# Robin-Lenoir/replication-social-bank-runs

Hardware: AMD Instinct MI355X
Metric: equilibria solved/sec on β×u grid (FP64) (higher is better)
Workload: dtype f64; 1 GPU; fig5_beta_u_sweep_2048x2048_per_gpu (BASELINE config 3); n_beta_per_gpu=2048, n_u=2048, early_exit=False, parallelism=beta-column shards x1, beta_axis_columns=2048, pipelined=True

## Files before the change

### include/sbr.h

```cpp
#ifndef SBR_H
#define SBR_H

#include <stdint.h>

#include "sbr_status.h"

#ifdef __cplusplus
extern "C" {
#endif

#define SBR_OK 0
#define SBR_EARG (-1)
#define SBR_EDEVICE (-2)
#define SBR_ENOMEM (-3)

typedef struct sbr_ctx sbr_ctx;

typedef struct {
    double ode_reltol;
    double ode_abstol;
    int64_t ode_maxiters;
    int32_t bisect_max_iters;
    int32_t early_exit_nan_run;
    int32_t knot_capacity;
    int32_t hetero_max_iters;
    int32_t flags;
    int32_t pad;
    double xi_guess;
} sbr_opts;

#define SBR_FLAG_EXHAUSTIVE 0x1
#define SBR_FLAG_READY_SWEEP 0x2
#define SBR_FLAG_RCCL_GATHER 0x4
#define SBR_FLAG_XI_GUESS 0x8
#define SBR_FLAG_DIAG_STOP_AFTER_BUFFER 0x100
#define SBR_FLAG_DIAG_STOP_AFTER_BISECT 0x200
#define SBR_FLAG_DIAG_COUNT_AW_BLOCKS 0x400
#define SBR_FLAG_DIAG_SOCIAL_PROF 0x800
#define SBR_FLAG_DIAG_NO_AW_WINDOW 0x1000
#define SBR_FLAG_HETERO_WIDE 0x2000

#define SBR_HETERO_MAX_K 16

typedef struct {
    double* xi;
    double* tau_in_unc;
    double* tau_out_unc;
    double* aw_max;
    double* tol;
    uint32_t* status;
    int32_t* iters;
} sbr_result_soa;

void sbr_default_opts(sbr_opts* o);

int sbr_init(int device, sbr_ctx** ctx);
int sbr_free(sbr_ctx* ctx);
const char* sbr_last_error(const sbr_ctx* ctx);

int sbr_init_multi(int n_gpus, const int* devices, sbr_ctx** ctx);
int sbr_multi_size(const sbr_ctx* ctx);
sbr_ctx* sbr_multi_child(sbr_ctx* ctx, int rank);

// ... 138 lines not shown
```

### replication-social-bank-runs_amd/csrc/sbr_baseline.hip

```cpp
#include "sbr_device.h"
#include "sbr_hazard_dev.h"
#include "sbr_kernels.h"
#include "sbr_ode.h"
#include "sbr_point_dev.h"
#include "sbr_scan.h"
#include "sbr_solve_dev.h"

namespace sbr {

constexpr int kLearnBlock = 128;
constexpr int kLearnBlockLat = 64;

__device__ __forceinline__ void publish_column(const LearnArgs& a, int b)
{
    const int k = atomicAdd(a.ready_tail, 1);
    __hip_atomic_store(a.ready_q + k, b + 1, __ATOMIC_RELEASE, __HIP_MEMORY_SCOPE_AGENT);
}
#define st_knot(p, v) (*(p) = (v))
constexpr int kStageSlots = 24;
constexpr size_t kStageLdsPerWave = (size_t)4 * kStageSlots * 64 * sizeof(double);
template <int LB, bool STAGE = false>
__global__ __launch_bounds__(LB) void learn_logistic_kernel(const double* __restrict__ beta,
                                                            const double* __restrict__ eta,
                                                            const double* __restrict__ t_end, LearnArgs a,
// ... 256 lines not shown
    double tin, tout;
    if (!any) {
        tin = T1; tout = T1;
    } else if (all) {
        tin = tau(0); tout = tau(ntau - 1);
    } else {
        tin = T1; tout = T1;
        if (cin >= 0) {
            const double t0 = tau(cin), t1 = tau(cin + 1), h0 = H[cin], h1 = H[cin + 1];
            tin = t0 + ((u - h0) * (t1 - t0)) / (h1 - h0);
        }
        if (cout >= 0) {
            const double t0 = tau(cout), t1 = tau(cout + 1), h0 = H[cout], h1 = H[cout + 1];
            tout = t0 + ((u - h0) * (t1 - t0)) / (h1 - h0);
        }
        if (tin == T1) tin = tau(fa);
        if (tout == T1) tout = tau(la);
    }
    r.tin = tin;
    r.tout = tout;
    if (diag & 1) return;
    solve_from_buffers(T, G, H, S, n, ntau, nle, ETA, T1, trunc, u, kappa, max_iters, lbits, r, aw_path, diag,
                       tin, tout);
}

template <class P>
__device__ __forceinline__ void solve_from_buffers(P T, P G, P H, const Summ& S, const int n, const int ntau,
                                                   const int nle, const double ETA, const double T1, const bool trunc,
                                                   const double u, const double kappa, const int max_iters,
                                                   const uint32_t lbits, PointResult& r, double* __restrict__ aw_path,
                                                   const int diag, const double tin, const double tout)
{
    const double tlo = T[0], thi = T[n - 1];
    auto tau = [&](int i) -> double { return i < nle ? T[i] : ETA; };
    if (tin == tout) {
        r.status = SBR_NO_RUN_HR_BELOW_U | SBR_CONVERGED | lbits;
        r.tol = 0.0;
        return;
    }

    uint32_t flag = 0;
    const double tolerance = 10.0 * sbr_jl_eps(kappa);
    double xnew = (tin + tout) / 2.0, xmin = tin, xmax = tout;
    const bool okmin = in_range(xmin, tlo, thi, trunc, flag);
    const bool okmax = in_range(xmax, tlo, thi, trunc, flag);
    if (!okmin || !okmax) {
// ... 410 lines not shown
        r.tin = NAN; r.tout = NAN;
        return;
    }
    sv.finish();
    const int ns = sv.nh;
    double tin, tout;
    if (!sv.any) {
        tin = T1; tout = T1;
    } else if (sv.all) {
        tin = tau[0]; tout = tau[ns - 1];
    } else {
        tin = sv.cin >= 0 ? sv.tin_x : T1;
        tout = sv.cout >= 0 ? sv.tout_x : T1;
        if (tin == T1) tin = tau[sv.fa];
        if (tout == T1) tout = tau[sv.la];
    }
    r.tin = tin;
    r.tout = tout;
    if (diag & 1) { r.status = bits; return; }
    solve_from_buffers(T, G, H, S, n, ntau, nle, ETA, T1, trunc, u, kappa, max_iters, bits, r, aw_path, diag, tin,
                       tout);
}

template <int BLOCK, bool INTEREST, int MODE = 0>
__device__ __forceinline__ void eq_column(const int b, const int j0, const int j1, const LearnBufs& L,
                                          const double* __restrict__ eta, const double* __restrict__ t_end,
                                          const double* __restrict__ u, const EqArgs& a, const InterestArgs& ia,
                                          const ResultSoA& out, double* smem)
{
    const int n = L.n_knots[b], ntau = L.n_tau[b], nle = L.n_le[b];
    const uint32_t lst = L.status[b];
    const size_t row = (size_t)b * (size_t)L.cap;
    const double* __restrict__ gT = L.t + row;
    const double* __restrict__ gG = L.G + row;
    const double* __restrict__ gH = L.hr + row;
    constexpr int NS = INTEREST ? 3 : 2;
    const bool fits = n <= a.lds_cap && (!INTEREST || ntau <= a.lds_cap);
    if ((MODE == 1 && !fits) || (MODE == 2 && fits)) return;
    double* sT = smem;
    double* sG = smem + a.lds_cap;
    double* sH = INTEREST ? smem + 2 * a.lds_cap : nullptr;
    const double* __restrict__ cH = INTEREST ? sH : gH;
    const int nsum = (a.lds_cap >> 6) + 1, nsum8 = (a.lds_cap >> 3) + 1;
    double* hmax = smem + NS * a.lds_cap;
    double* hmin = hmax + nsum;
    double* pmc = hmin + nsum;
    double* smc = pmc + nsum8;
    double* hpm = smc + nsum8;
    double* hpn = hpm + nsum;
    double* hsm = hpn + nsum;
    double* hsn = hsm + nsum;
    const int nbh_s = (ntau + 63) >> 6;
    __shared__ int eq_next;
    __shared__ int s_nonmono;
    __shared__ int s_noscan;
    __shared__ int s_near1;
    __shared__ int s_ndec;
    __shared__ unsigned long long s_maxdec;
    __shared__ double s_thalf;
    __shared__ int s_wb;
    __shared__ unsigned long long s_dmax;
    if (threadIdx.x == 0) { eq_next = 0; s_nonmono = 0; s_noscan = 0; s_near1 = 0; s_ndec = 0; s_maxdec = 0; s_thalf = NAN; s_wb = 0x7fffffff; s_dmax = 0; }
    if (fits) {
        for (int i = threadIdx.x; i < n; i += BLOCK) { sT[i] = gT[i]; sG[i] = gG[i]; }
        if (INTEREST)
            for (int i = threadIdx.x; i < ntau; i += BLOCK) sH[i] = gH[i];
    }
    __syncthreads();
    Summ S{nullptr, nullptr, nullptr, nullptr, false, (double)NAN, false, 0.0, false, 2, nullptr, nullptr, nullptr,
           nullptr, 0};
    if (fits && !a.exhaustive) {
        const int nbh = (ntau + 63) >> 6, nbg = (n + 7) >> 3;
        const int nq = nbh << 3;
        for (int bk = threadIdx.x; bk < nq + nbg; bk += BLOCK) {
            if (bk < nq) {
                double mx = -INFINITY, mn = INFINITY;
                const int i0 = bk << 3;
                double h[8];
#pragma unroll
                for (int k = 0; k < 8; k++) h[k] = i0 + k < ntau ? cH[i0 + k] : -INFINITY;
#pragma unroll
                for (int k = 0; k < 8; k++) {
                    if (i0 + k >= ntau) continue;
                    if (h[k] > mx) mx = h[k];
                    mn = (h[k] != h[k]) ? -INFINITY : (h[k] < mn ? h[k] : mn);
                }
#pragma unroll
                for (int off = 1; off < 8; off <<= 1) {
                    const double omx = __shfl_xor(mx, off, 8), omn = __shfl_xor(mn, off, 8);
                    mx = omx > mx ? omx : mx;
                    mn = omn < mn ? omn : mn;
                }
                if ((bk & 7) == 0) {
                    hmax[bk >> 3] = mx;
                    hmin[bk >> 3] = mn;
                }
            } else {
                const int g = bk - nq;
                double mx = -INFINITY, mn = INFINITY;
                const int e = (g << 3) + 8 < n ? (g << 3) + 8 : n;
                double prev = g > 0 ? sG[(g << 3) - 1] : -INFINITY;
                bool mono = true, nan = false;
                int ndec = 0;
                double maxdec = 0.0;
                for (int i = g << 3; i < e; i++) {
                    const double v = sG[i];
                    if (v != v) { mx = NAN; mn = NAN; mono = false; nan = true; break; }
                    if (v > mx) mx = v;
                    if (v < mn) mn = v;
                    const bool dec = v < prev;
                    mono &= !dec;
                    ndec += dec ? 1 : 0;
                    maxdec = dec && prev - v > maxdec ? prev - v : maxdec;
                    prev = v;
                }
                if (!mono) s_nonmono = 1;
                if (nan) s_noscan = 1;
                if (ndec) {
                    atomicAdd(&s_ndec, ndec);
                    atomicMax(&s_maxdec, (unsigned long long)sbr_dbits(maxdec));
                }
                const double sep = 1e-15 * sT[n - 1];
                bool far = true, far1 = true;
                for (int i = g << 3; i < e; i++) {
                    far &= i + 2 >= n || sT[i + 2] - sT[i] > sep;
                    far1 &= i + 1 >= n || sT[i + 1] - sT[i] > sep;
                }
                if (!far) s_noscan = 1;
                if (!far1) s_near1 = 1;
                pmc[g] = mx;
                smc[g] = mn;
            }
        }
        {
            auto rises = [](double lo, double hi) {
                const double m = fabs(lo) > fabs(hi) ? fabs(lo) : fabs(hi);
                return m >= 0x1p-900 && m <= 1e300 && hi - lo > 0x1p-50 * m;
            };
            const int ln = threadIdx.x & 63;
            for (int q = threadIdx.x >> 6; q * 62 < n - 1; q += BLOCK >> 6) {
                const int k = q * 62 + ln - 2;
                const bool valid = k >= 0 && k <= n - 2;
                const double d = valid ? (sG[k + 1] - sG[k]) / (sT[k + 1] - sT[k]) : 0.0;
                const double d1 = __shfl_up(d, 1, 64);
                const bool inc = rises(d1, d), dec = rises(d, d1);
                const bool incp = __shfl_up((int)inc, 1, 64) != 0;
                const bool mine = valid && ln >= 2;
                const bool fail = mine && k >= 1 && ((!inc && !dec) || (k >= 2 && inc && !incp));
                double ad = mine ? fabs(d) : 0.0;
                ad = ad <= 1e300 ? ad : (double)INFINITY;
#pragma unroll
                for (int off = 1; off < 64; off <<= 1) {
                    const double o = __shfl_xor(ad, off, 64);
                    ad = o > ad ? o : ad;
                }
                const unsigned long long fm = __ballot(fail);
                if (ln == 0) {
                    if (fm) atomicMin(&s_wb, q * 62 + (int)__builtin_ctzll(fm) - 2);
                    atomicMax(&s_dmax, (unsigned long long)sbr_dbits(ad));
                }
            }
        }
        __syncthreads();
        if (threadIdx.x == 0) {
            int lo = 0, hi = n - 1;
            if (n >= 2 && sG[0] <= 0.5 && sG[n - 1] > 0.5) {
                while (hi - lo > 1) {
                    const int mid = (lo + hi) >> 1;
                    if (sG[mid] <= 0.5) lo = mid;
                    else hi = mid;
                }
                s_thalf = sT[lo] + (0.5 - sG[lo]) * (sT[hi] - sT[lo]) / (sG[hi] - sG[lo]);
            }
            if (s_nonmono && s_noscan)
            for (int g = 1; g < nbg; g++) {
                const double a0 = pmc[g - 1], b0 = pmc[g];
                pmc[g] = (a0 != a0 || b0 != b0) ? NAN : (a0 > b0 ? a0 : b0);
            }
        } else if (threadIdx.x == (BLOCK > 64 ? 64 : 1) && s_nonmono && s_noscan) {
            for (int g = nbg - 2; g >= 0; g--) {
                const double a0 = smc[g + 1], b0 = smc[g];
                smc[g] = (a0 != a0 || b0 != b0) ? NAN : (a0 < b0 ? a0 : b0);
            }
        }
        if (BLOCK >= 256 && (threadIdx.x >> 6) >= 2 && (threadIdx.x >> 6) <= 3) {
            const bool fwd = (threadIdx.x >> 6) == 2;
            const int ln = threadIdx.x & 63;
            double ca = -INFINITY, cb = INFINITY;
            for (int c0 = 0; c0 < nbh; c0 += 64) {
                const int g = fwd ? c0 + ln : nbh - 1 - c0 - ln;
                const bool in = fwd ? g < nbh : g >= 0;
                double a = in ? hmax[g] : -INFINITY, b = in ? hmin[g] : INFINITY;
                for (int off = 1; off < 64; off <<= 1) {
                    const double oa = __shfl_up(a, off, 64), ob = __shfl_up(b, off, 64);
                    if (ln >= off) { a = oa > a ? oa : a; b = ob < b ? ob : b; }
                }
                a = ca > a ? ca : a;
                b = cb < b ? cb : b;
                if (in) {
                    if (fwd) { hpm[g] = a; hpn[g] = b; }
                    else { hsm[g] = a; hsn[g] = b; }
                }
                ca = __shfl(a, 63, 64);
                cb = __shfl(b, 63, 64);
            }
        }
        if (BLOCK < 256 && threadIdx.x == 2) {
            double a0 = -INFINITY, b0 = INFINITY;
            for (int g = 0; g < nbh; g++) {
                a0 = hmax[g] > a0 ? hmax[g] : a0;
                b0 = hmin[g] < b0 ? hmin[g] : b0;
                hpm[g] = a0;
                hpn[g] = b0;
            }
        }
        if (BLOCK < 256 && threadIdx.x == 3) {
            double a0 = -INFINITY, b0 = INFINITY;
            for (int g = nbh - 1; g >= 0; g--) {
                a0 = hmax[g] > a0 ? hmax[g] : a0;
                b0 = hmin[g] < b0 ? hmin[g] : b0;
                hsm[g] = a0;
                hsn[g] = b0;
            }
        }
        __syncthreads();
        auto uni = [](double x) {
            const unsigned long long v = sbr_dbits(x);
            const unsigned lo = __builtin_amdgcn_readfirstlane((unsigned)v);
            const unsigned hi = __builtin_amdgcn_readfirstlane((unsigned)(v >> 32));
            return sbr_bitsd(((unsigned long long)hi << 32) | lo);
        };
        const double dd = uni((double)s_ndec * sbr_bitsd(s_maxdec));
        S = Summ{hmax, hmin, pmc, smc, s_nonmono == 0, uni(s_thalf),
                 n >= 2 && !s_noscan && dd <= 1e-12 && sG[0] >= 0.0 && sG[n - 1] <= 2.0, dd,
                 s_nonmono == 0 || s_noscan != 0, s_near1 == 0 ? 1 : 2,
                 hpm, hpn, hsm, hsn, nbh_s};
        const double dmax = sbr_bitsd(s_dmax);
        if (n >= 2 && dmax <= 1e300 && !(a.diag & 16)) {
            const int wb = s_wb < n - 1 ? s_wb : n - 1;
            const double e0 = fabs(sT[0]), e1 = fabs(sT[n - 1]);
            const double span = (sT[wb] + 2.0 * (e0 > e1 ? e0 : e1)) * (1.0 + 0x1p-40);
            const double du = 0x1p-52 * span;
            const double wm = 0x1p-46 + dmax * (0x1p-50 * span);
            if (wm <= 1e-9) {
                S.wlo = uni((sT[0] > 0.0 ? sT[0] : 0.0) + du);
                S.whi = uni(sT[wb] - du);
                S.wm = uni(wm);
            }
        }
    }
    const int lane = threadIdx.x & 63;
    const double ETA = eta[b], T1 = t_end[b];
    const uint32_t lbits = lst & (SBR_ODE_MAXITERS | SBR_STIFF_SWITCH | SBR_ODE_FAILED | SBR_KNOT_OVERFLOW);
    const bool bad_col = (lst & (SBR_ARG_INVALID | SBR_OOB)) || n < 2;
    const bool trunc = !a.full_grid && n >= 2 && gT[n - 1] < T1 && !(lst & kLearnCutBits);
    for (;;) {
        int base = 0;
        if (lane == 0) base = atomicAdd(&eq_next, 64);
        base = __builtin_amdgcn_readfirstlane(base);
        if (j0 + base >= j1) break;
        const int j = j0 + base + lane;
        if (j >= j1) continue;
        const double uj = u[j];
        PointResult r;
        int64_t vsteps = 0;
        if (bad_col || !(uj >= 0.0)) {
            r.xi = NAN; r.aw = NAN; r.tol = INFINITY; r.iters = 0;
            r.tin = NAN; r.tout = NAN;
            r.status = ((lst & SBR_ARG_INVALID) || !(uj >= 0.0)) ? SBR_ARG_INVALID : (SBR_OOB | lbits);
        } else if (INTEREST && ia.r > 0.0) {
            if (MODE != 2 && fits)
                solve_interest_point(sT, sG, sH, S, n, ntau, nle, ETA, T1, trunc, uj, a.kappa, a.max_iters, lbits, ia,
                                     r, vsteps, a.aw_path, a.diag);
            else if (MODE != 1)
                solve_interest_point(gT, gG, gH, S, n, ntau, nle, ETA, T1, trunc, uj, a.kappa, a.max_iters, lbits, ia,
                                     r, vsteps, a.aw_path, a.diag);
        } else if (MODE != 2 && fits) {
            solve_point((const double*)sT, (const double*)sG, cH, S, n, ntau, nle, ETA, T1, trunc, uj, a.kappa,
// ... 229 lines not shown

hipError_t launch_learn_logistic(const double* beta, const double* eta, const double* t_end, const LearnArgs& a,
                                 const LearnBufs& L, hipStream_t s)
{
    hipError_t e = launch_learn_kernel(beta, eta, t_end, a, L, s, (a.fuse_hazard && !a.ready_q) ? 0 : 1);
    if (e != hipSuccess) return e;
    if (a.ready_q) return hipSuccess;
    if (a.fuse_hazard) return launch_hazard_norm(a, L, a.n_beta, s);
    hipLaunchKernelGGL(hazard_kernel, dim3(a.n_beta), dim3(HZ_BLOCK), 0, s, beta,
                       eta, a, L);
    return hipGetLastError();
}

hipError_t launch_hazard(const double* beta, const double* eta, const LearnArgs& a, const LearnBufs& L, int n_beta,
                         hipStream_t s)
{
    hipLaunchKernelGGL(hazard_kernel, dim3(n_beta), dim3(HZ_BLOCK), 0, s, beta, eta, a, L);
    return hipGetLastError();
}

hipError_t launch_equilibrium(const LearnBufs& L, const double* eta, const double* t_end, const double* u,
                              const EqArgs& a, const ResultSoA& out, int n_beta, hipStream_t s, int only_mode)
{
    const size_t lds = ((size_t)2 * a.lds_cap + 6 * ((a.lds_cap >> 6) + 1) + 2 * ((a.lds_cap >> 3) + 1)) * sizeof(double);
    const int tiles = (a.n_u + EQ_TILE - 1) / EQ_TILE;
    const int w = a.n_u < EQ_TILE ? a.n_u : EQ_TILE;
    dim3 grid(tiles, n_beta);
    const InterestArgs none{0.0, 1.0, 0.0, 0.0, 0, nullptr, nullptr, nullptr};
    auto go = [&](auto k1, auto k2, int bs) {
        if (only_mode != 2) hipLaunchKernelGGL(k1, grid, dim3(bs), lds, s, L, eta, t_end, u, a, none, out);
        if (only_mode != 1) hipLaunchKernelGGL(k2, grid, dim3(bs), 0, s, L, eta, t_end, u, a, none, out);
    };
    if (w > 256)
        go(equilibrium_kernel<kEqWide, false, 1>, equilibrium_kernel<kEqWide, false, 2>, kEqWide);
    else if (w > 64)
        go(equilibrium_kernel<256, false, 1>, equilibrium_kernel<256, false, 2>, 256);
    else
        go(equilibrium_kernel<64, false, 1>, equilibrium_kernel<64, false, 2>, 64);
    return hipGetLastError();
}

hipError_t launch_eq_ready(const LearnBufs& L, const double* beta, const double* eta, const double* t_end,
                           const double* u, const LearnArgs& la, const EqArgs& a, const ReadyArgs& ra,
                           const ResultSoA& out, int n_blocks, hipStream_t s)
{
    size_t lds = ((size_t)2 * a.lds_cap + 6 * ((a.lds_cap >> 6) + 1) + 2 * ((a.lds_cap >> 3) + 1)) * sizeof(double);
    const size_t hz = (size_t)(3 * HZ_LDS + 3) * sizeof(double);
    if (lds < hz) lds = hz;
    (void)n_blocks;
    hipLaunchKernelGGL(eq_ready_kernel, dim3(ra.n_items), dim3(kEqWide), lds, s, L, beta, eta, t_end, u, la, a, ra,
                       out);
    return hipGetLastError();
}

__global__ __launch_bounds__(256) void ready_fail_kernel(const int32_t* __restrict__ gave_up, ResultSoA out,
                                                          int64_t n_pts)
{
    if (__hip_atomic_load(gave_up, __ATOMIC_RELAXED, __HIP_MEMORY_SCOPE_AGENT) == 0) return;
    for (int64_t i = (int64_t)blockIdx.x * 256 + threadIdx.x; i < n_pts; i += (int64_t)gridDim.x * 256) {
        out.xi[i] = NAN;
        out.tau_in_unc[i] = NAN;
        out.tau_out_unc[i] = NAN;
        out.aw_max[i] = NAN;
        out.tol[i] = INFINITY;
        out.status[i] = SBR_ENGINE_SCHED;
        if (out.iters) out.iters[i] = 0;
    }
}

hipError_t launch_ready_fail(const int32_t* gave_up, const ResultSoA& out, int64_t n_pts, hipStream_t s)
{
    hipLaunchKernelGGL(ready_fail_kernel, dim3(256), dim3(256), 0, s, gave_up, out, n_pts);
// ... 37 lines not shown
```

### replication-social-bank-runs_amd/csrc/sbr_capi.hip

```cpp
#include <math.h>
#include <stdio.h>
#include <stdlib.h>
#include <string.h>

#include <algorithm>
#include <array>
#include <chrono>
#include <string>
#include <thread>
#include <vector>

#include "../../include/sbr.h"
#include "../../include/sbr_detmath.h"
#include "sbr_hostcopy.h"
#include "sbr_kernels.h"
#include "sbr_multi.h"
#include "sbr_social_plan.h"

constexpr unsigned kTimingEventFlags = hipEventDisableSystemFence;
constexpr unsigned kSyncEventFlags = hipEventDisableTiming | hipEventReleaseToDevice;



struct sbr_ctx {
// ... 377 lines not shown

hipEvent_t tstart(sbr_ctx* c, hipStream_t s)
{
    if (!c->timing) return nullptr;
    hipEvent_t e = next_event(c);
    if (e) (void)hipEventRecord(e, s);
    return e;
}

void tend(sbr_ctx* c, hipStream_t s, int kind, hipEvent_t a, int count = 1)
{
    if (!c->timing || !a) return;
    hipEvent_t e = next_event(c);
    if (!e) return;
    (void)hipEventRecord(e, s);
    c->trec.push_back({kind, a, e, count});
}

int launch_eq(sbr_ctx* c, hipStream_t s, const sbr::LearnBufs& L, const double* eta, const double* t_end,
              const double* u, int64_t n_beta, int64_t n_u, double kappa, const sbr_opts& o,
              const sbr::ResultSoA& out, double* aw_path, int group = 1, bool timed = true)
{
    sbr::EqArgs ea{kappa, (int32_t)n_u, o.bisect_max_iters, c->lds_cap_b, aw_path,
                   (o.flags & SBR_FLAG_EXHAUSTIVE) ? 1 : 0, (o.flags >> 8) & 0x17};
    ea.group = group;
    hipEvent_t t0 = timed ? tstart(c, s) : nullptr;
    if (aw_path && n_beta == 1 && n_u == 1) {
        ea.lds_cap = c->lds_cap;
        HIP_TRY(c, sbr::launch_point_coop(L, eta, t_end, u, ea, out, s), SBR_EDEVICE);
        tend(c, s, 1, t0);
        return SBR_OK;
    }
    HIP_TRY(c, sbr::launch_equilibrium(L, eta, t_end, u, ea, out, (int)n_beta, s), SBR_EDEVICE);
    tend(c, s, 1, t0);
    return SBR_OK;
}

int ensure_pipe_streams(sbr_ctx* c)
{
    if (c->lstream[0]) return SBR_OK;
    int lo = 0, hi = 0;
    (void)hipDeviceGetStreamPriorityRange(&lo, &hi);
    for (int k = 0; k < sbr_ctx::kLearnStreams; k++)
        HIP_TRY(c, hipStreamCreateWithPriority(&c->lstream[k], hipStreamNonBlocking, hi), SBR_EDEVICE);
    for (int k = 0; k < sbr_ctx::kLearnSlots; k++) {
        HIP_TRY(c, hipEventCreateWithFlags(&c->ev_learned[k], kSyncEventFlags), SBR_EDEVICE);
        HIP_TRY(c, hipEventCreateWithFlags(&c->ev_eq[k], kSyncEventFlags), SBR_EDEVICE);
// ... 100 lines not shown
        c->rq_cap = need;
    }
    return SBR_OK;
}

int run_baseline_ready(sbr_ctx* c, hipStream_t s, const double* beta, const double* eta, const double* t_end,
                       const double* u, int64_t n_beta, int64_t n_u, double kappa, const sbr_opts& o,
                       sbr::LearnArgs la, const sbr::ResultSoA& out)
{
    const int tiles = (int)((n_u + kReadyTileU - 1) / kReadyTileU);
    int32_t* q = c->rq;
    HIP_TRY(c, hipEventRecord(c->ev_rin, s), SBR_EDEVICE);
    HIP_TRY(c, hipStreamWaitEvent(c->rs_learn, c->ev_rin, 0), SBR_EDEVICE);
    HIP_TRY(c, hipMemsetAsync(q, 0, (4 + 2 * (size_t)n_beta) * 4, c->rs_learn), SBR_EDEVICE);
    HIP_TRY(c, hipEventRecord(c->ev_rq, c->rs_learn), SBR_EDEVICE);
    HIP_TRY(c, hipStreamWaitEvent(c->rs_eq, c->ev_rq, 0), SBR_EDEVICE);
    la.fuse_hazard = 0;
    la.ready_tail = q + 2;
    la.ready_q = q + 4;
    hipEvent_t t0 = tstart(c, c->rs_learn);
    HIP_TRY(c, sbr::launch_learn_logistic(beta, eta, t_end, la, c->LW[0], c->rs_learn), SBR_EDEVICE);
    tend(c, c->rs_learn, 0, t0);
    sbr::EqArgs ea{kappa, (int32_t)n_u, o.bisect_max_iters, c->lds_cap_b, nullptr,
                   (o.flags & SBR_FLAG_EXHAUSTIVE) ? 1 : 0, (o.flags >> 8) & 0x17};
    sbr::ReadyArgs ra{q, q + 4, q + 4 + n_beta, (int32_t)(n_beta * tiles), tiles, kReadyTileU, kReadySpin};
    hipEvent_t t1 = tstart(c, c->rs_eq);
    HIP_TRY(c, sbr::launch_eq_ready(c->LW[0], beta, eta, t_end, u, la, ea, ra, out, 0, c->rs_eq), SBR_EDEVICE);
    tend(c, c->rs_eq, 1, t1);
    HIP_TRY(c, hipEventRecord(c->ev_rl, c->rs_learn), SBR_EDEVICE);
    HIP_TRY(c, hipEventRecord(c->ev_re, c->rs_eq), SBR_EDEVICE);
    HIP_TRY(c, hipStreamWaitEvent(s, c->ev_rl, 0), SBR_EDEVICE);
    HIP_TRY(c, hipStreamWaitEvent(s, c->ev_re, 0), SBR_EDEVICE);
    HIP_TRY(c, sbr::launch_ready_fail(q + 1, out, n_beta * n_u, s), SBR_EDEVICE);
    return SBR_OK;
}

int run_baseline(sbr_ctx* c, hipStream_t s, const double* beta, const double* eta, const double* t_end, double x0,
                 const double* u, int64_t n_beta, int64_t n_u, double p, double kappa, double lambda,
                 const sbr_opts& o, const sbr::ResultSoA& out, double* aw_path)
{
    int rc = ensure_learn(c, (size_t)n_beta, (size_t)o.knot_capacity);
    if (rc) return rc;
    c->last_slot = 0;
    c->last_off = 0;
    sbr::LearnArgs la{x0, o.ode_reltol, o.ode_abstol, p, lambda, o.ode_maxiters, (int32_t)n_beta, stop_after_eta(o), 0};
    c->rs_used = !aw_path && n_beta >= 64 && (o.flags & SBR_FLAG_READY_SWEEP) &&
                 ensure_ready(c, (size_t)n_beta) == SBR_OK;
// ... 14 lines not shown
        const int64_t wk = waves >> (kSweepChunks - k);
        lo[k] = std::min<int64_t>(n_beta, std::max<int64_t>(wk * 64, (int64_t)k * 64));
    }
    lo[1] = std::min<int64_t>(lo[2] - 64, std::max<int64_t>(64, (waves / kSweepFront) * 64));
    HIP_TRY(c, hipEventRecord(c->ev_in, s), SBR_EDEVICE);
    hipEvent_t t0 = tstart(c, s);
    c->ck_start = c->timing ? t0 : nullptr;
    c->ck_ev.assign(c->timing ? 2 * kSweepChunks : 0, nullptr);
    for (int k = 0; k < kSweepChunks; k++) {
        hipStream_t ls = c->lstream[k];
        const int64_t c0 = lo[k], nb = lo[k + 1] - lo[k];
        HIP_TRY(c, hipStreamWaitEvent(ls, c->ev_in, 0), SBR_EDEVICE);
        if (nb <= 0) continue;
        sbr::LearnArgs lk = la;
        lk.n_beta = (int32_t)nb;
        const sbr::LearnBufs Lk = learn_rows(c->LW[0], (size_t)c0);
        HIP_TRY(c, sbr::launch_learn_logistic(beta + c0, eta + c0, t_end + c0, lk, Lk, ls), SBR_EDEVICE);
        if (c->timing) {
            c->ck_ev[2 * k] = next_event(c);
            if (c->ck_ev[2 * k]) (void)hipEventRecord(c->ck_ev[2 * k], ls);
        }
        HIP_TRY(c, hipEventRecord(c->ev_learned[k], ls), SBR_EDEVICE);
        sbr::EqArgs ea{kappa, (int32_t)n_u, o.bisect_max_iters, c->lds_cap_b, nullptr,
                       (o.flags & SBR_FLAG_EXHAUSTIVE) ? 1 : 0, (o.flags >> 8) & 0x17};
        HIP_TRY(c, sbr::launch_equilibrium(Lk, eta + c0, t_end + c0, u, ea, result_rows(out, (size_t)(c0 * n_u)),
                                           (int)nb, ls), SBR_EDEVICE);
        if (c->timing) {
            c->ck_ev[2 * k + 1] = next_event(c);
            if (c->ck_ev[2 * k + 1]) (void)hipEventRecord(c->ck_ev[2 * k + 1], ls);
        }
        HIP_TRY(c, hipEventRecord(c->ev_eq[k], ls), SBR_EDEVICE);
    }
    for (int k = 0; k < kSweepChunks; k++)
        if (lo[k + 1] > lo[k]) HIP_TRY(c, hipStreamWaitEvent(s, c->ev_learned[k], 0), SBR_EDEVICE);
    hipEvent_t t1 = tstart(c, s);
    tend(c, s, 0, t0);
    for (int k = 0; k < kSweepChunks; k++)
        if (lo[k + 1] > lo[k]) HIP_TRY(c, hipStreamWaitEvent(s, c->ev_eq[k], 0), SBR_EDEVICE);
    tend(c, s, 1, t1);
    return SBR_OK;
}

size_t point_bytes(size_t cap) { return 4 * cap * sizeof(double) + 6 * sizeof(int32_t); }

int run_points(sbr_ctx* c, hipStream_t s, const double* beta, const double* eta, const double* t_end, double x0,
               const double* u, const double* p, const double* kappa, const double* lambda, int64_t n,
               const sbr_opts& o, const sbr::ResultSoA& out)
// ... 27 lines not shown
        const sbr::PointArgs pa{beta + c0, eta + c0,    t_end + c0,         u + c0,    p + c0,
                                kappa + c0, lambda + c0, o.bisect_max_iters, c->lds_cap};
        t0 = tstart(c, s);
        HIP_TRY(c, sbr::launch_points(L, la, pa, result_rows(out, (size_t)c0), (int)nc, s), SBR_EDEVICE);
        tend(c, s, 1, t0);
    }
    return SBR_OK;
}

int run_interest(sbr_ctx* c, hipStream_t s, const double* beta, const double* eta, const double* t_end, double x0,
                 const double* u, int64_t n_beta, int64_t n_u, double p, double kappa, double lambda, double r,
                 double delta, const sbr_opts& o, const sbr::ResultSoA& out, int64_t* steps, double* aw_path = nullptr,
                 double* v_path = nullptr, int32_t* v_count = nullptr)
{
    int rc = ensure_learn(c, (size_t)n_beta, (size_t)o.knot_capacity);
    if (rc) return rc;
    c->last_slot = 0;
    c->last_off = 0;
    sbr::LearnArgs la{x0, o.ode_reltol, o.ode_abstol, p, lambda, o.ode_maxiters, (int32_t)n_beta, stop_after_eta(o), 0};
    hipEvent_t t0 = tstart(c, s);
    HIP_TRY(c, sbr::launch_learn_logistic(beta, eta, t_end, la, c->LW[0], s), SBR_EDEVICE);
    tend(c, s, 0, t0);
    sbr::EqArgs ea{kappa, (int32_t)n_u, o.bisect_max_iters, c->lds_cap, aw_path,
                   (o.flags & SBR_FLAG_EXHAUSTIVE) ? 1 : 0, (o.flags >> 8) & 0x17};
    sbr::InterestArgs ia{r, delta, o.ode_reltol, o.ode_abstol, o.ode_maxiters, steps, v_path, v_count};
    t0 = tstart(c, s);
    HIP_TRY(c, sbr::launch_interest(c->LW[0], eta, t_end, u, ea, ia, out, (int)n_beta, s), SBR_EDEVICE);
    tend(c, s, 1, t0);
    return SBR_OK;
}

bool interest_valid(double r, double delta) { return r >= 0.0 && delta > 0.0 && r < delta; }

int multi_sweep_social(sbr_ctx* c, const double* beta, const double* eta, double x0, const double* u, int64_t n_beta,
                       int64_t n_u, double p, double kappa, double lambda, const double* cmp_grid, int32_t n_cmp,
                       double tol, int32_t max_iter, const sbr_opts& o, sbr_result_soa* out, int32_t* fp_iters,
                       int64_t* rk_steps);
int multi_sweep_hetero(sbr_ctx* c, int32_t K, const double* betas, const double* dist, const double* eta,
                       const double* t_end, double x0, const double* u, int64_t n_col, int64_t n_u, double p,
                       double kappa, double lambda, const sbr_opts& o, sbr_result_soa* out, double* tau_in,
                       double* tau_out);
int multi_sweep_interest(sbr_ctx* c, const double* beta, const double* eta, const double* t_end, double x0,
                         const double* u, int64_t n_beta, int64_t n_u, double p, double kappa, double lambda, double r_,
                         double delta, const sbr_opts& o, sbr_result_soa* out, int64_t* rk_steps);
int multi_sweep_baseline(sbr_ctx* c, const double* beta, const double* eta, const double* t_end, double x0,
                         const double* u, int64_t n_beta, int64_t n_u, double p, double kappa, double lambda,
                         const sbr_opts& o, sbr_result_soa* out);
// ... 961 lines not shown
            double* hs = (double*)(H + K.sc);
            hs[0] = beta;
            hs[1] = eta;
            memcpy(H + K.tg, t, (size_t)n * 8);
            memcpy(H + K.tg + (size_t)n * 8, G, (size_t)n * 8);
            if (pdf) memcpy(H + K.tg + (size_t)n * 16, pdf, (size_t)n * 8);
            HIP_TRY(c, hipMemcpyAsync(D, H, K.tg + (size_t)n * (pdf ? 24 : 16), hipMemcpyHostToDevice, s), SBR_EDEVICE);
            sbr::LearnArgs la{0.0, o.ode_reltol, o.ode_abstol, p, lambda, o.ode_maxiters, 1, 0, 0, nullptr, nullptr};
            la.pdf = pdf ? dtg + 2 * n : nullptr;
            HIP_TRY(c, sbr::launch_hazard(dsc, dsc + 1, la, L, 1, s), SBR_EDEVICE);
            if (ntau > 0)
                HIP_TRY(c, hipMemcpyAsync(H + K.hr, D + K.hr, (size_t)ntau * 8, hipMemcpyDeviceToHost, s), SBR_EDEVICE);
            HIP_TRY(c, hipMemcpyAsync(H, D, 32, hipMemcpyDeviceToHost, s), SBR_EDEVICE);
        }
        const size_t nu = (size_t)n_u;
        if (n_u == 1) {
            double* z = c->kn_zc;
            double* zd = c->kn_zc_dev;
            z[0] = t_end;
            z[1] = u[0];
            const sbr::ResultSoA r{zd + 2, zd + 3, zd + 4, zd + 5, zd + 6, (uint32_t*)(zd + 7), (int32_t*)(zd + 7) + 1};
            double* zp = zd + 16;
            sbr::EqArgs ea{kappa, 1, o.bisect_max_iters, c->lds_cap, want_aw ? zp : nullptr,
                           (o.flags & SBR_FLAG_EXHAUSTIVE) ? 1 : 0, (o.flags >> 8) & 0x17,
                           want_aw ? zp + ntau : nullptr, want_aw ? zp + 2 * ntau : nullptr, 1, dres};
            if (o.flags & SBR_FLAG_XI_GUESS) ea.xi_guess = o.xi_guess;
            HIP_TRY(c, sbr::launch_point_coop(L, dsc + 1, zd, zd + 1, ea, r, s), SBR_EDEVICE);
        } else {
            double* hu = (double*)(H + K.u);
            hu[0] = t_end;
            memcpy(hu + 1, u, nu * 8);
            HIP_TRY(c, hipMemcpyAsync(du, hu, (nu + 1) * 8, hipMemcpyHostToDevice, s), SBR_EDEVICE);
            const sbr::ResultSoA r{dres, dres + nu, dres + 2 * nu, dres + 3 * nu, dres + 4 * nu,
                                   (uint32_t*)(dres + 5 * nu), (int32_t*)(dres + 5 * nu) + nu};
            if ((o.flags & SBR_FLAG_XI_GUESS) && o.xi_guess == o.xi_guess) {
                sbr::EqArgs ea{kappa, 1, o.bisect_max_iters, c->lds_cap, nullptr,
                               (o.flags & SBR_FLAG_EXHAUSTIVE) ? 1 : 0, (o.flags >> 8) & 0x17, nullptr, nullptr, 1};
                ea.xi_guess = o.xi_guess;
                HIP_TRY(c, sbr::launch_point_coop(L, dsc + 1, du, du + 1, ea, r, s, (int)nu), SBR_EDEVICE);
            } else {
                sbr::EqArgs ea{kappa, (int32_t)n_u, o.bisect_max_iters, c->lds_cap_b, nullptr,
                               (o.flags & SBR_FLAG_EXHAUSTIVE) ? 1 : 0, (o.flags >> 8) & 0x17, nullptr, nullptr, 1};
                HIP_TRY(c, sbr::launch_equilibrium(L, dsc + 1, du, du + 1, ea, r, 1, s, n <= c->lds_cap_b ? 1 : 2),
                        SBR_EDEVICE);
            }
            HIP_TRY(c, hipMemcpyAsync(H + K.res, D + K.res, res_bytes, hipMemcpyDeviceToHost, s), SBR_EDEVICE);
        }
        HIP_TRY(c, hipStreamSynchronize(s), SBR_EDEVICE);
        return SBR_OK;
    });
    if (rc) return rc;
    if (!hit) {
        const int32_t* hc = (const int32_t*)H;
        if (hc[1] != (int32_t)ntau) return fail(c, SBR_EDEVICE, "hazard grid length mismatch");
        c->kn_t.assign(t, t + n);
        c->kn_G.assign(G, G + n);
        if (pdf) c->kn_pdf.assign(pdf, pdf + n);
        else c->kn_pdf.clear();
        const double* hh = (const double*)(H + K.hr);
        c->kn_hr.assign(hh, hh + ntau);
        memcpy(c->kn_key, key, sizeof key);
        c->kn_n = n;
        c->kn_m = (int32_t)m;
        c->kn_ntau = (int32_t)ntau;
        c->kn_valid = true;
// ... 1075 lines not shown
```

### replication-social-bank-runs_amd/sbr/_lib.py

```python
from __future__ import annotations

import ctypes
import os
import re
from pathlib import Path

PKG_ROOT = Path(__file__).resolve().parent.parent
REPO_ROOT = PKG_ROOT.parent
LIB_PATH = Path(os.environ["SBR_LIB"]) if os.environ.get("SBR_LIB") else PKG_ROOT / "lib" / "libsbr.so"
HEADER = REPO_ROOT / "include" / "sbr.h"
STATUS_HEADER = REPO_ROOT / "include" / "sbr_status.h"

_D = ctypes.c_double
_I64 = ctypes.c_int64
_I32 = ctypes.c_int32
_P = ctypes.c_void_p

SBR_OK, SBR_EARG, SBR_EDEVICE, SBR_ENOMEM = 0, -1, -2, -3
SBR_FLAG_EXHAUSTIVE = 0x1
SBR_FLAG_READY_SWEEP = 0x2
SBR_FLAG_RCCL_GATHER = 0x4
SBR_FLAG_XI_GUESS = 0x8
SBR_FLAG_DIAG_STOP_AFTER_BUFFER = 0x100
SBR_FLAG_DIAG_STOP_AFTER_BISECT = 0x200
SBR_FLAG_DIAG_COUNT_AW_BLOCKS = 0x400
SBR_FLAG_DIAG_SOCIAL_PROF = 0x800
SBR_FLAG_DIAG_NO_AW_WINDOW = 0x1000
SBR_FLAG_HETERO_WIDE = 0x2000
SBR_HETERO_MAX_K = 16


class SBRNativeError(RuntimeError):
    """The native engine is unavailable or returned an error."""


class ArgumentError(ValueError):
    """Mirror of Julia's ArgumentError raised by the reference's constructors."""


class Opts(ctypes.Structure):
    _fields_ = [
        ("ode_reltol", _D),
        ("ode_abstol", _D),
        ("ode_maxiters", _I64),
        ("bisect_max_iters", _I32),
        ("early_exit_nan_run", _I32),
        ("knot_capacity", _I32),
        ("hetero_max_iters", _I32),
        ("flags", _I32),
        ("pad", _I32),
        ("xi_guess", _D),
# ... 136 lines not shown
```

Baseline: 6.110 billion equilibria/s.

## Split equilibrium column into buffer-time pass then lazy G staging and solves

```diff
diff --git a/include/sbr.h b/include/sbr.h
--- a/include/sbr.h
+++ b/include/sbr.h
@@ -39,6 +39,7 @@
 #define SBR_FLAG_DIAG_SOCIAL_PROF 0x800
 #define SBR_FLAG_DIAG_NO_AW_WINDOW 0x1000
 #define SBR_FLAG_HETERO_WIDE 0x2000
+#define SBR_FLAG_DIAG_STOP_AFTER_STAGING 0x4000
 
 #define SBR_HETERO_MAX_K 16
 
diff --git a/replication-social-bank-runs_amd/csrc/sbr_baseline.hip b/replication-social-bank-runs_amd/csrc/sbr_baseline.hip
--- a/replication-social-bank-runs_amd/csrc/sbr_baseline.hip
+++ b/replication-social-bank-runs_amd/csrc/sbr_baseline.hip
@@ -302,6 +302,48 @@
     if (diag & 1) return;
     solve_from_buffers(T, G, H, S, n, ntau, nle, ETA, T1, trunc, u, kappa, max_iters, lbits, r, aw_path, diag,
                        tin, tout);
+}
+
+template <class P, class SU, class Q>
+__device__ __forceinline__ void buffer_times_bs(P T, P H, const SU& S, Q hpm, Q hpn, Q hsm, Q hsn, const int nb,
+                                                const int ntau, const int nle, const double ETA, const double T1,
+                                                const double u, double& tin, double& tout)
+{
+    auto blk_end = [&](int b) { return (b << 6) + 64 < ntau ? (b << 6) + 64 : ntau; };
+    auto tau = [&](int i) -> double { return i < nle ? T[i] : ETA; };
+    tin = T1; tout = T1;
+    const int ba = bs_first_gt_inc(hpm, nb, u);
+    const int fa = ba < nb ? scan_fwd<true>(H, ba << 6, blk_end(ba), u) : -1;
+    if (fa < 0) return;
+    const int bb = bs_first_le_dec(hpn, nb, u);
+    const int fb = bb < nb ? scan_fwd<false>(H, bb << 6, blk_end(bb), u) : -1;
+    if (fb < 0) { tin = tau(0); tout = tau(ntau - 1); return; }
+    const int lab = bs_last_gt_dec(hsm, nb, u);
+    const int la = lab >= 0 ? scan_bwd<true>(H, lab << 6, blk_end(lab) - 1, u) : -1;
+    int cin, cout;
+    if (fa > 0) {
+        cin = fa - 1;
+    } else {
+        const int k = first_above(H, S, ntau, fb, u);
+        cin = k >= 0 ? k - 1 : -1;
+    }
+    if (la < ntau - 1) {
+        cout = la;
+    } else {
+        const int lbb = bs_last_le_inc(hsn, nb, u);
+        const int lb = lbb >= 0 ? scan_bwd<false>(H, lbb << 6, blk_end(lbb) - 1, u) : -1;
+        cout = last_above(H, S, lb, u);
+    }
+    if (cin >= 0) {
+        const double t0 = tau(cin), t1 = tau(cin + 1), h0 = H[cin], h1 = H[cin + 1];
+        tin = t0 + ((u - h0) * (t1 - t0)) / (h1 - h0);
+    }
+    if (cout >= 0) {
+        const double t0 = tau(cout), t1 = tau(cout + 1), h0 = H[cout], h1 = H[cout + 1];
+        tout = t0 + ((u - h0) * (t1 - t0)) / (h1 - h0);
+    }
+    if (tin == T1) tin = tau(fa);
+    if (tout == T1) tout = tau(la);
 }
 
 template <class P>
@@ -758,6 +800,8 @@
                        tout);
 }
 
+constexpr size_t kEqCtlBytes = (EQ_TILE / 64) * sizeof(unsigned long long) + 16;
+
 template <int BLOCK, bool INTEREST, int MODE = 0>
 __device__ __forceinline__ void eq_column(const int b, const int j0, const int j1, const LearnBufs& L,
                                           const double* __restrict__ eta, const double* __restrict__ t_end,
@@ -771,7 +815,7 @@
     const double* __restrict__ gG = L.G + row;
     const double* __restrict__ gH = L.hr + row;
     constexpr int NS = INTEREST ? 3 : 2;
-    const bool fits = n <= a.lds_cap && (!INTEREST || ntau <= a.lds_cap);
+    const bool fits = n <= a.lds_cap && ntau <= a.lds_cap;
     if ((MODE == 1 && !fits) || (MODE == 2 && fits)) return;
     double* sT = smem;
     double* sG = smem + a.lds_cap;
@@ -797,24 +841,20 @@
     __shared__ int s_wb;
     __shared__ unsigned long long s_dmax;
     if (threadIdx.x == 0) { eq_next = 0; s_nonmono = 0; s_noscan = 0; s_near1 = 0; s_ndec = 0; s_maxdec = 0; s_thalf = NAN; s_wb = 0x7fffffff; s_dmax = 0; }
-    if (fits) {
-        for (int i = threadIdx.x; i < n; i += BLOCK) { sT[i] = gT[i]; sG[i] = gG[i]; }
-        if (INTEREST)
-            for (int i = threadIdx.x; i < ntau; i += BLOCK) sH[i] = gH[i];
-    }
-    __syncthreads();
-    Summ S{nullptr, nullptr, nullptr, nullptr, false, (double)NAN, false, 0.0, false, 2, nullptr, nullptr, nullptr,
-           nullptr, 0};
-    if (fits && !a.exhaustive) {
-        const int nbh = (ntau + 63) >> 6, nbg = (n + 7) >> 3;
-        const int nq = nbh << 3;
-        for (int bk = threadIdx.x; bk < nq + nbg; bk += BLOCK) {
-            if (bk < nq) {
+    const int nbh = (ntau + 63) >> 6, nbg = (n + 7) >> 3;
+    auto hr_blocks = [&](auto copy, const double* __restrict__ src, double* dst) {
+        constexpr bool COPY = decltype(copy)::value;
+        for (int bk = threadIdx.x; bk < (nbh << 3); bk += BLOCK) {
                 double mx = -INFINITY, mn = INFINITY;
                 const int i0 = bk << 3;
                 double h[8];
 #pragma unroll
-                for (int k = 0; k < 8; k++) h[k] = i0 + k < ntau ? cH[i0 + k] : -INFINITY;
+                for (int k = 0; k < 8; k++) h[k] = i0 + k < ntau ? src[i0 + k] : -INFINITY;
+                if constexpr (COPY) {
+#pragma unroll
+                    for (int k = 0; k < 8; k++)
+                        if (i0 + k < ntau) dst[i0 + k] = h[k];
+                }
 #pragma unroll
                 for (int k = 0; k < 8; k++) {
                     if (i0 + k >= ntau) continue;
@@ -831,8 +871,10 @@
                     hmax[bk >> 3] = mx;
                     hmin[bk >> 3] = mn;
                 }
-            } else {
-                const int g = bk - nq;
+        }
+    };
+    auto g_blocks = [&]() {
+        for (int g = threadIdx.x; g < nbg; g += BLOCK) {
                 double mx = -INFINITY, mn = INFINITY;
                 const int e = (g << 3) + 8 < n ? (g << 3) + 8 : n;
                 double prev = g > 0 ? sG[(g << 3) - 1] : -INFINITY;
@@ -866,7 +908,6 @@
                 if (!far1) s_near1 = 1;
                 pmc[g] = mx;
                 smc[g] = mn;
-            }
         }
         {
             auto rises = [](double lo, double hi) {
@@ -897,7 +938,8 @@
                 }
             }
         }
-        __syncthreads();
+    };
+    auto g_tables = [&]() {
         if (threadIdx.x == 0) {
             int lo = 0, hi = n - 1;
             if (n >= 2 && sG[0] <= 0.5 && sG[n - 1] > 0.5) {
@@ -919,6 +961,8 @@
                 smc[g] = (a0 != a0 || b0 != b0) ? NAN : (a0 < b0 ? a0 : b0);
             }
         }
+    };
+    auto hr_tables = [&]() {
         if (BLOCK >= 256 && (threadIdx.x >> 6) >= 2 && (threadIdx.x >> 6) <= 3) {
             const bool fwd = (threadIdx.x >> 6) == 2;
             const int ln = threadIdx.x & 63;
@@ -959,7 +1003,8 @@
                 hsn[g] = b0;
             }
         }
-        __syncthreads();
+    };
+    auto make_summ = [&]() {
         auto uni = [](double x) {
             const unsigned long long v = sbr_dbits(x);
             const unsigned lo = __builtin_amdgcn_readfirstlane((unsigned)v);
@@ -967,7 +1012,7 @@
             return sbr_bitsd(((unsigned long long)hi << 32) | lo);
         };
         const double dd = uni((double)s_ndec * sbr_bitsd(s_maxdec));
-        S = Summ{hmax, hmin, pmc, smc, s_nonmono == 0, uni(s_thalf),
+        Summ S{hmax, hmin, pmc, smc, s_nonmono == 0, uni(s_thalf),
                  n >= 2 && !s_noscan && dd <= 1e-12 && sG[0] >= 0.0 && sG[n - 1] <= 2.0, dd,
                  s_nonmono == 0 || s_noscan != 0, s_near1 == 0 ? 1 : 2,
                  hpm, hpn, hsm, hsn, nbh_s};
@@ -984,12 +1029,125 @@
                 S.wm = uni(wm);
             }
         }
-    }
+        return S;
+    };
     const int lane = threadIdx.x & 63;
     const double ETA = eta[b], T1 = t_end[b];
     const uint32_t lbits = lst & (SBR_ODE_MAXITERS | SBR_STIFF_SWITCH | SBR_ODE_FAILED | SBR_KNOT_OVERFLOW);
     const bool bad_col = (lst & (SBR_ARG_INVALID | SBR_OOB)) || n < 2;
     const bool trunc = !a.full_grid && n >= 2 && gT[n - 1] < T1 && !(lst & kLearnCutBits);
+    if constexpr (!INTEREST && MODE != 2) {
+        if (fits && !a.exhaustive) {
+            struct HrSumm { const double *hmax, *hmin; };
+            const HrSumm HS{hmax, hmin};
+            double* sHR = sG;
+            unsigned long long* s_cand = reinterpret_cast<unsigned long long*>(hsn + nsum);
+            int& eq_next2 = reinterpret_cast<int*>(s_cand + EQ_TILE / 64)[0];
+            int& s_anyc = reinterpret_cast<int*>(s_cand + EQ_TILE / 64)[1];
+            if (threadIdx.x == 0) { eq_next2 = 0; s_anyc = 0; }
+            for (int i = threadIdx.x; i < n; i += BLOCK) sT[i] = gT[i];
+            hr_blocks(BoolC<true>{}, gH, sHR);
+            __syncthreads();
+            hr_tables();
+            __syncthreads();
+            const bool points = !(a.diag & 64);
+            while (points) {
+                int base = 0;
+                if (lane == 0) base = atomicAdd(&eq_next, 64);
+                base = __builtin_amdgcn_readfirstlane(base);
+                if (j0 + base >= j1) break;
+                const int j = j0 + base + lane;
+                bool cand = false;
+                if (j < j1) {
+                    const double uj = u[j];
+                    PointResult r;
+                    r.xi = NAN; r.aw = NAN; r.tol = INFINITY; r.iters = 0; r.status = 0;
+                    if (bad_col || !(uj >= 0.0)) {
+                        r.tin = NAN; r.tout = NAN;
+                        r.status = ((lst & SBR_ARG_INVALID) || !(uj >= 0.0)) ? SBR_ARG_INVALID : (SBR_OOB | lbits);
+                    } else {
+                        buffer_times_bs((const double*)sT, (const double*)sHR, HS, (const double*)hpm,
+                                        (const double*)hpn, (const double*)hsm, (const double*)hsn, nbh, ntau, nle,
+                                        ETA, T1, uj, r.tin, r.tout);
+                        if (!(a.diag & 1)) {
+                            if (r.tin == r.tout) {
+                                r.status = SBR_NO_RUN_HR_BELOW_U | SBR_CONVERGED | lbits;
+                                r.tol = 0.0;
+                            } else {
+                                cand = true;
+                            }
+                        }
+                    }
+                    const size_t o = (size_t)b * (size_t)a.n_u + j;
+                    out.tau_in_unc[o] = r.tin;
+                    out.tau_out_unc[o] = r.tout;
+                    if (!cand) {
+                        out.xi[o] = r.xi;
+                        out.aw_max[o] = r.aw;
+                        out.tol[o] = r.tol;
+                        out.status[o] = r.status;
+                        if (out.iters) out.iters[o] = r.iters;
+                    }
+                }
+                const unsigned long long m = __ballot(cand);
+                s_cand[base >> 6] = m;
+                if (m) s_anyc = 1;
+            }
+            __syncthreads();
+            const bool solves = s_anyc != 0;
+            if (solves || (a.diag & (1 | 64))) {
+                for (int i = threadIdx.x; i < n; i += BLOCK) sG[i] = gG[i];
+                __syncthreads();
+                g_blocks();
+                __syncthreads();
+                g_tables();
+                __syncthreads();
+                const Summ S = make_summ();
+                while (solves) {
+                    int base = 0;
+                    if (lane == 0) base = atomicAdd(&eq_next2, 64);
+                    base = __builtin_amdgcn_readfirstlane(base);
+                    if (j0 + base >= j1) break;
+                    const unsigned long long m = s_cand[base >> 6];
+                    const unsigned mlo = __builtin_amdgcn_readfirstlane((unsigned)m);
+                    const unsigned mhi = __builtin_amdgcn_readfirstlane((unsigned)(m >> 32));
+                    if ((mlo | mhi) == 0) continue;
+                    if (!(((lane < 32 ? mlo : mhi) >> (lane & 31)) & 1u)) continue;
+                    const int j = j0 + base + lane;
+                    const size_t o = (size_t)b * (size_t)a.n_u + j;
+                    const double uj = u[j];
+                    PointResult r;
+                    r.xi = NAN; r.aw = NAN; r.tol = INFINITY; r.iters = 0; r.status = 0;
+                    solve_from_buffers((const double*)sT, (const double*)sG, (const double*)nullptr, S, n, ntau, nle,
+                                       ETA, T1, trunc, uj, a.kappa, a.max_iters, lbits, r, a.aw_path, a.diag,
+                                       out.tau_in_unc[o], out.tau_out_unc[o]);
+                    out.xi[o] = r.xi;
+                    out.aw_max[o] = r.aw;
+                    out.tol[o] = r.tol;
+                    out.status[o] = r.status;
+                    if (out.iters) out.iters[o] = r.iters;
+                }
+            }
+            return;
+        }
+    }
+    if (fits) {
+        for (int i = threadIdx.x; i < n; i += BLOCK) { sT[i] = gT[i]; sG[i] = gG[i]; }
+        if (INTEREST)
+            for (int i = threadIdx.x; i < ntau; i += BLOCK) sH[i] = gH[i];
+    }
+    __syncthreads();
+    Summ S{nullptr, nullptr, nullptr, nullptr, false, (double)NAN, false, 0.0, false, 2, nullptr, nullptr, nullptr,
+           nullptr, 0};
+    if (INTEREST && fits && !a.exhaustive) {
+        hr_blocks(BoolC<false>{}, cH, nullptr);
+        g_blocks();
+        __syncthreads();
+        g_tables();
+        hr_tables();
+        __syncthreads();
+        S = make_summ();
+    }
     for (;;) {
         int base = 0;
         if (lane == 0) base = atomicAdd(&eq_next, 64);
@@ -1265,7 +1423,8 @@
 hipError_t launch_equilibrium(const LearnBufs& L, const double* eta, const double* t_end, const double* u,
                               const EqArgs& a, const ResultSoA& out, int n_beta, hipStream_t s, int only_mode)
 {
-    const size_t lds = ((size_t)2 * a.lds_cap + 6 * ((a.lds_cap >> 6) + 1) + 2 * ((a.lds_cap >> 3) + 1)) * sizeof(double);
+    const size_t lds = ((size_t)2 * a.lds_cap + 6 * ((a.lds_cap >> 6) + 1) + 2 * ((a.lds_cap >> 3) + 1)) * sizeof(double) +
+                       kEqCtlBytes;
     const int tiles = (a.n_u + EQ_TILE - 1) / EQ_TILE;
     const int w = a.n_u < EQ_TILE ? a.n_u : EQ_TILE;
     dim3 grid(tiles, n_beta);
@@ -1287,10 +1446,12 @@
                            const double* u, const LearnArgs& la, const EqArgs& a, const ReadyArgs& ra,
                            const ResultSoA& out, int n_blocks, hipStream_t s)
 {
-    size_t lds = ((size_t)2 * a.lds_cap + 6 * ((a.lds_cap >> 6) + 1) + 2 * ((a.lds_cap >> 3) + 1)) * sizeof(double);
+    size_t lds = ((size_t)2 * a.lds_cap + 6 * ((a.lds_cap >> 6) + 1) + 2 * ((a.lds_cap >> 3) + 1)) * sizeof(double) +
+                       kEqCtlBytes;
     const size_t hz = (size_t)(3 * HZ_LDS + 3) * sizeof(double);
     if (lds < hz) lds = hz;
     (void)n_blocks;
+    if (ra.tile_u > EQ_TILE) return hipErrorInvalidValue;
     hipLaunchKernelGGL(eq_ready_kernel, dim3(ra.n_items), dim3(kEqWide), lds, s, L, beta, eta, t_end, u, la, a, ra,
                        out);
     return hipGetLastError();
diff --git a/replication-social-bank-runs_amd/csrc/sbr_capi.hip b/replication-social-bank-runs_amd/csrc/sbr_capi.hip
--- a/replication-social-bank-runs_amd/csrc/sbr_capi.hip
+++ b/replication-social-bank-runs_amd/csrc/sbr_capi.hip
@@ -423,7 +423,7 @@
               const sbr::ResultSoA& out, double* aw_path, int group = 1, bool timed = true)
 {
     sbr::EqArgs ea{kappa, (int32_t)n_u, o.bisect_max_iters, c->lds_cap_b, aw_path,
-                   (o.flags & SBR_FLAG_EXHAUSTIVE) ? 1 : 0, (o.flags >> 8) & 0x17};
+                   (o.flags & SBR_FLAG_EXHAUSTIVE) ? 1 : 0, (o.flags >> 8) & 0x57};
     ea.group = group;
     hipEvent_t t0 = timed ? tstart(c, s) : nullptr;
     if (aw_path && n_beta == 1 && n_u == 1) {
@@ -570,7 +570,7 @@
     HIP_TRY(c, sbr::launch_learn_logistic(beta, eta, t_end, la, c->LW[0], c->rs_learn), SBR_EDEVICE);
     tend(c, c->rs_learn, 0, t0);
     sbr::EqArgs ea{kappa, (int32_t)n_u, o.bisect_max_iters, c->lds_cap_b, nullptr,
-                   (o.flags & SBR_FLAG_EXHAUSTIVE) ? 1 : 0, (o.flags >> 8) & 0x17};
+                   (o.flags & SBR_FLAG_EXHAUSTIVE) ? 1 : 0, (o.flags >> 8) & 0x57};
     sbr::ReadyArgs ra{q, q + 4, q + 4 + n_beta, (int32_t)(n_beta * tiles), tiles, kReadyTileU, kReadySpin};
     hipEvent_t t1 = tstart(c, c->rs_eq);
     HIP_TRY(c, sbr::launch_eq_ready(c->LW[0], beta, eta, t_end, u, la, ea, ra, out, 0, c->rs_eq), SBR_EDEVICE);
@@ -631,7 +631,7 @@
         }
         HIP_TRY(c, hipEventRecord(c->ev_learned[k], ls), SBR_EDEVICE);
         sbr::EqArgs ea{kappa, (int32_t)n_u, o.bisect_max_iters, c->lds_cap_b, nullptr,
-                       (o.flags & SBR_FLAG_EXHAUSTIVE) ? 1 : 0, (o.flags >> 8) & 0x17};
+                       (o.flags & SBR_FLAG_EXHAUSTIVE) ? 1 : 0, (o.flags >> 8) & 0x57};
         HIP_TRY(c, sbr::launch_equilibrium(Lk, eta + c0, t_end + c0, u, ea, result_rows(out, (size_t)(c0 * n_u)),
                                            (int)nb, ls), SBR_EDEVICE);
         if (c->timing) {
@@ -705,7 +705,7 @@
     HIP_TRY(c, sbr::launch_learn_logistic(beta, eta, t_end, la, c->LW[0], s), SBR_EDEVICE);
     tend(c, s, 0, t0);
     sbr::EqArgs ea{kappa, (int32_t)n_u, o.bisect_max_iters, c->lds_cap, aw_path,
-                   (o.flags & SBR_FLAG_EXHAUSTIVE) ? 1 : 0, (o.flags >> 8) & 0x17};
+                   (o.flags & SBR_FLAG_EXHAUSTIVE) ? 1 : 0, (o.flags >> 8) & 0x57};
     sbr::InterestArgs ia{r, delta, o.ode_reltol, o.ode_abstol, o.ode_maxiters, steps, v_path, v_count};
     t0 = tstart(c, s);
     HIP_TRY(c, sbr::launch_interest(c->LW[0], eta, t_end, u, ea, ia, out, (int)n_beta, s), SBR_EDEVICE);
@@ -1713,7 +1713,7 @@
             const sbr::ResultSoA r{zd + 2, zd + 3, zd + 4, zd + 5, zd + 6, (uint32_t*)(zd + 7), (int32_t*)(zd + 7) + 1};
             double* zp = zd + 16;
             sbr::EqArgs ea{kappa, 1, o.bisect_max_iters, c->lds_cap, want_aw ? zp : nullptr,
-                           (o.flags & SBR_FLAG_EXHAUSTIVE) ? 1 : 0, (o.flags >> 8) & 0x17,
+                           (o.flags & SBR_FLAG_EXHAUSTIVE) ? 1 : 0, (o.flags >> 8) & 0x57,
                            want_aw ? zp + ntau : nullptr, want_aw ? zp + 2 * ntau : nullptr, 1, dres};
             if (o.flags & SBR_FLAG_XI_GUESS) ea.xi_guess = o.xi_guess;
             HIP_TRY(c, sbr::launch_point_coop(L, dsc + 1, zd, zd + 1, ea, r, s), SBR_EDEVICE);
@@ -1726,12 +1726,12 @@
                                    (uint32_t*)(dres + 5 * nu), (int32_t*)(dres + 5 * nu) + nu};
             if ((o.flags & SBR_FLAG_XI_GUESS) && o.xi_guess == o.xi_guess) {
                 sbr::EqArgs ea{kappa, 1, o.bisect_max_iters, c->lds_cap, nullptr,
-                               (o.flags & SBR_FLAG_EXHAUSTIVE) ? 1 : 0, (o.flags >> 8) & 0x17, nullptr, nullptr, 1};
+                               (o.flags & SBR_FLAG_EXHAUSTIVE) ? 1 : 0, (o.flags >> 8) & 0x57, nullptr, nullptr, 1};
                 ea.xi_guess = o.xi_guess;
                 HIP_TRY(c, sbr::launch_point_coop(L, dsc + 1, du, du + 1, ea, r, s, (int)nu), SBR_EDEVICE);
             } else {
                 sbr::EqArgs ea{kappa, (int32_t)n_u, o.bisect_max_iters, c->lds_cap_b, nullptr,
-                               (o.flags & SBR_FLAG_EXHAUSTIVE) ? 1 : 0, (o.flags >> 8) & 0x17, nullptr, nullptr, 1};
+                               (o.flags & SBR_FLAG_EXHAUSTIVE) ? 1 : 0, (o.flags >> 8) & 0x57, nullptr, nullptr, 1};
                 HIP_TRY(c, sbr::launch_equilibrium(L, dsc + 1, du, du + 1, ea, r, 1, s, n <= c->lds_cap_b ? 1 : 2),
                         SBR_EDEVICE);
             }
diff --git a/replication-social-bank-runs_amd/sbr/_lib.py b/replication-social-bank-runs_amd/sbr/_lib.py
--- a/replication-social-bank-runs_amd/sbr/_lib.py
+++ b/replication-social-bank-runs_amd/sbr/_lib.py
@@ -27,6 +27,7 @@
 SBR_FLAG_DIAG_SOCIAL_PROF = 0x800
 SBR_FLAG_DIAG_NO_AW_WINDOW = 0x1000
 SBR_FLAG_HETERO_WIDE = 0x2000
+SBR_FLAG_DIAG_STOP_AFTER_STAGING = 0x4000
 SBR_HETERO_MAX_K = 16
 
 
```

Result: slower. 5.956 billion equilibria/s (-2.5%).
